# the-professor510/RSMCRT

Hardware: AMD Instinct MI355X
Metric: photon packets/sec (128^3 jmean grid, path-length deposition) (higher is better)
Workload: dtype f64

## Files before the change

include/smcrt.h:

```cpp
#ifndef SMCRT_H
#define SMCRT_H

#include <stddef.h>
#include <stdint.h>

#ifdef __cplusplus
extern "C" {
#endif

#define SMCRT_ABI_VERSION 5

typedef enum smcrt_status {
  SMCRT_OK = 0,
  SMCRT_ERR_INVALID_ARG = -1,
  SMCRT_ERR_HIP = -2,
  SMCRT_ERR_RCCL = -3,
  SMCRT_ERR_DEVICE_FAULT = -4,
  SMCRT_ERR_NO_DEVICE = -5,
  SMCRT_ERR_OOM = -6,
  SMCRT_ERR_UNSUPPORTED = -7
} smcrt_status;

typedef enum smcrt_sdf_kind {
  SMCRT_SDF_SPHERE = 1,
// ... 321 lines not shown
  int64_t lean_hazards;
} smcrt_kernel_times;

int smcrt_scene_set_timing(smcrt_scene* scene, int32_t enable);
int smcrt_scene_kernel_times(smcrt_scene* scene, smcrt_kernel_times* out);

enum {
  SMCRT_DEPOSIT_ATOMIC = 0,
  SMCRT_DEPOSIT_SORTED = 1,
  SMCRT_DEPOSIT_BUCKETS = 2
};
int smcrt_scene_deposit_regime(const smcrt_scene* scene, int32_t* regime);

int smcrt_scene_invoxel_segments(smcrt_scene* scene, int64_t* out);

int smcrt_normalise_fluence(float* grid, const smcrt_grid* g, uint64_t nphotons);

typedef enum smcrt_symmetry {
  SMCRT_SYM_NONE = 0,
  SMCRT_SYM_PRISM = 1,
  SMCRT_SYM_FLIPPED = 2,
  SMCRT_SYM_UNIFORM_SLAB = 3,
  SMCRT_SYM_NONE_ROTATIONAL = 4,
  SMCRT_SYM_ROTATIONAL_360 = 5
} smcrt_symmetry;

typedef struct smcrt_escape_config {
  int32_t symmetry;
  int32_t n[3];
  double max[3];
// ... 131 lines not shown
```

rsmcrt_amd/abi.py:

```python
import ctypes as C

SMCRT_ABI_VERSION = 5

OK = 0
ERR_INVALID_ARG = -1
ERR_HIP = -2
ERR_RCCL = -3
ERR_DEVICE_FAULT = -4
ERR_NO_DEVICE = -5
ERR_OOM = -6
ERR_UNSUPPORTED = -7

STATUS_NAMES = {
    OK: "OK", ERR_INVALID_ARG: "INVALID_ARG", ERR_HIP: "HIP_ERROR", ERR_RCCL: "RCCL_ERROR",
    ERR_DEVICE_FAULT: "DEVICE_FAULT", ERR_NO_DEVICE: "NO_DEVICE", ERR_OOM: "OUT_OF_MEMORY",
    ERR_UNSUPPORTED: "UNSUPPORTED",
}

SDF_SPHERE, SDF_BOX, SDF_TORUS, SDF_CYLINDER, SDF_TRIPRISM = 1, 2, 3, 4, 5
SDF_SEGMENT, SDF_CAPSULE, SDF_CONE, SDF_EGG, SDF_PLANE, SDF_MODEL = 6, 7, 8, 9, 10, 11
SDF_REVOLUTION, SDF_EXTRUDE, SDF_ONION, SDF_TWIST, SDF_BEND, SDF_ELONGATE, SDF_DISPLACEMENT = 12, 13, 14, 15, 16, 17, 18
DISP_SINE, DISP_EXPR = 1, 2

OP_UNION, OP_SMOOTH_UNION, OP_SUBTRACTION, OP_INTERSECTION = 0, 1, 2, 3
# ... 208 lines not shown
EXPORTED_SYMBOLS = [
    "smcrt_abi_version", "smcrt_device_count", "smcrt_last_error", "smcrt_scene_create",
    "smcrt_scene_destroy", "smcrt_scene_det_bins", "smcrt_scene_set_optprops", "smcrt_run",
    "smcrt_run_device", "smcrt_normalise_fluence", "smcrt_scene_set_timing", "smcrt_scene_kernel_times",
    "smcrt_write_data_f32", "smcrt_write_data_f64", "smcrt_write_detector", "smcrt_write_checkpoint",
    "smcrt_job_load", "smcrt_job_destroy", "smcrt_job_info", "smcrt_job_scene", "smcrt_job_metadata", "smcrt_job_run",
    "smcrt_scene_info", "smcrt_run_origins", "smcrt_scene_classify", "smcrt_escape_sym_dims", "smcrt_escape_cells",
    "smcrt_escape_map", "smcrt_escape_run", "smcrt_scene_get_optprops", "smcrt_inverse_run", "smcrt_job_load_mode",
    "smcrt_job_escape_config", "smcrt_job_inverse_config", "smcrt_job_targets", "smcrt_job_run_escape",
    "smcrt_job_run_inverse", "smcrt_scene_fence",
    "smcrt_pack_size", "smcrt_pack_host", "smcrt_unpack_host", "smcrt_comm_unique_id", "smcrt_comm_init_rank",
    "smcrt_comm_info", "smcrt_comm_destroy", "smcrt_reduce_device_tallies", "smcrt_multi_create", "smcrt_multi_info",
    "smcrt_multi_scene", "smcrt_multi_run", "smcrt_multi_accumulate", "smcrt_multi_collect",
    "smcrt_multi_device_photons", "smcrt_multi_destroy", "smcrt_job_run_devices",
    "smcrt_spectral_sample", "smcrt_scene_set_spectral", "smcrt_scene_check",
    "smcrt_scene_invoxel_segments",
    "smcrt_scene_set_path_tracking", "smcrt_scene_path_counts", "smcrt_scene_read_paths", "smcrt_write_paths",
    "smcrt_job_history_filename",
    "smcrt_scene_set_phasor", "smcrt_scene_read_phasor", "smcrt_scene_reset_phasor",
    "smcrt_displacement_compile", "smcrt_displacement_eval", "smcrt_displacement_describe",
    "smcrt_voxel_scene_create", "smcrt_scene_deposit_regime",
]
```

rsmcrt_amd/csrc/sceneplan.cpp:

```cpp
#include "sceneplan.h"

#include <algorithm>
#include <cmath>
#include <cstdlib>
#include <cstring>
#include <functional>
#include <string>

#include "dispexpr.h"
#include "hosterr.h"

namespace smcrt {
namespace {

int fail(int code, const std::string& msg) { return set_error(code, msg); }
bool is(const char* v, const char* s) { return v && std::strcmp(v, s) == 0; }

}

Knobs read_knobs() {
  Knobs k;
  auto num = [](const char* v, double d) { return v ? std::atof(v) : d; };
  if (const char* cm = std::getenv("SMCRT_COOP_MIN_TOPS")) k.coop_min_tops = std::max(1, std::atoi(cm));
  if (const char* cl = std::getenv("SMCRT_COOP_LANES")) k.coop_lanes = std::max(1, std::min(64, std::atoi(cl)));
// ... 6 lines not shown
  k.cull_grid.u_frac = num(std::getenv("SMCRT_CULL_UFRAC"), 1.0);
  k.cull_log = std::getenv("SMCRT_CULL_LOG") != nullptr;
  k.far_march = !is(std::getenv("SMCRT_FAR_MARCH"), "0");
  const char* dm = std::getenv("SMCRT_DEPOSIT");
  k.deposit_atomic = is(dm, "atomic");
  k.deposit_sorted = is(dm, "sorted");
  if (const char* pc = std::getenv("SMCRT_POOL_CAP"))
    k.pool_cap_chunks = std::max<uint64_t>(1, std::strtoull(pc, nullptr, 10) / CHUNK_RECORDS);
  const char* fp = std::getenv("SMCRT_FOLD_PRIO");
  k.fold_prio = !(fp && fp[0] == '0');
  k.fused_hist = !is(std::getenv("SMCRT_FUSED_HIST"), "0");
  const char* wsl = std::getenv("SMCRT_WS_SLOTS");
  k.ws_two_slots = wsl && wsl[0] == '2';
  const char* wi = std::getenv("SMCRT_WS_INVOXEL");
  k.ws_invoxel = wi ? (is(wi, "0") ? 0 : 1) : -1;
  const char* le = std::getenv("SMCRT_LEAN");
  k.lean_mode = le ? (is(le, "0") ? 0 : 1) : -1;
  const char* lm = std::getenv("SMCRT_DEBUG_LEAN_MARGIN");
  k.lean_debug = is(lm, "all") ? 2u : (is(lm, "0") ? 1u : 0u);
  k.verbose = std::getenv("SMCRT_VERBOSE") != nullptr;
  return k;
}

LaunchKnobs read_launch_knobs() {
  LaunchKnobs k;
#ifdef SMCRT_DIAG
  const char* dd = std::getenv("SMCRT_DIAG_DONE");
  k.diag_done = dd && dd[0] == '1';
#endif
  if (const char* wm = std::getenv("SMCRT_WATCHDOG_MS")) k.watchdog_ms = std::strtod(wm, nullptr);
// ... 241 lines not shown
  if (!p.ctab.empty() || p.cull.enabled) plan_far_march(nodes, top, n_top, grid, knobs.far_march, p);
  plan_grid_mode(grid, p);
  plan_deposit(grid, knobs, p);
  p.face_bytes = p.faces.size() * sizeof(double) + sizeof(TopProps) * (size_t)n_top;
  p.lds_faces = p.face_bytes <= MAX_FACE_BYTES;
  for (int32_t i = 1; i < n_top; ++i) p.fresnel = p.fresnel || p.h_props[i].n != p.h_props[0].n;
  {
    bool ok = p.bucketed && p.coop_lanes == 0 && grid->nx < (1 << 20) - 2 && grid->ny < (1 << 20) - 2 &&
              grid->nz < (1 << 20) - 2;
    p.ws_slots = (!knobs.ws_two_slots && lean_lds(p) + lim.ws_shared3 <= LDS_BYTES) ? 3 : 2;
    ok = ok && lean_lds(p) + (p.ws_slots == 3 ? lim.ws_shared3 : lim.ws_shared2) <= LDS_BYTES;
    p.lean_mode = knobs.lean_mode;
    p.lean_candidate = ok && !p.nested && (p.lean_mode == 1 || (p.lean_mode != 0 && n_dets == 0));
    p.lean_debug = knobs.lean_debug;
    p.ws_invoxel = knobs.ws_invoxel;
  }
  p.fold_prio = knobs.fold_prio;
  p.cull_log = knobs.cull_log;
  p.verbose = knobs.verbose;
  return SMCRT_OK;
}

int plan_voxel_scene(const uint8_t* labels, const smcrt_medium* media, int32_t n_media, const smcrt_grid* grid,
                     const smcrt_detector* dets, int32_t n_dets, const Knobs& knobs, ScenePlan* out) {
  if (!labels || !media || !grid || n_dets < 0 || (n_dets > 0 && !dets))
    return fail(SMCRT_ERR_INVALID_ARG, "voxel scene: NULL argument");
  if (n_media < 1 || n_media > 256)
    return fail(SMCRT_ERR_INVALID_ARG, "voxel scene: n_media = " + std::to_string(n_media) + " is outside 1 .. 256");
  if (grid->nx < 1 || grid->ny < 1 || grid->nz < 1 || !(grid->xmax > 0) || !(grid->ymax > 0) || !(grid->zmax > 0) ||
      !std::isfinite(grid->xmax) || !std::isfinite(grid->ymax) || !std::isfinite(grid->zmax))
// ... 63 lines not shown
```

rsmcrt_amd/csrc/sceneplan.h:

```cpp
#pragma once
#include <stdint.h>

#include <algorithm>
#include <vector>

#include "../../include/smcrt.h"
#include "transport.h"
#include "cull.h"
#include "deposit.h"

namespace smcrt {

constexpr int MAX_SLOTS = 4;
#ifndef SMCRT_DEEP_SLOT_GIB
#define SMCRT_DEEP_SLOT_GIB 24
#endif
constexpr uint64_t DEEP_SLOT_BYTES = (uint64_t)SMCRT_DEEP_SLOT_GIB << 30;

enum QueueWord : int {
  Q_STREAM0 = 0,
  Q_CALLER = MAX_SLOTS,
  Q_FAR_STEPS,
  Q_FOLD_TICKS,
  Q_LEAN_HAZARDS,
  Q_WATCHDOG,
  Q_INVOXEL,
  Q_COUNT
};
constexpr int N_QUEUES = Q_CALLER + 1;

constexpr size_t LDS_BYTES = 163840;
constexpr size_t MAX_FACE_BYTES = 40960;
constexpr uint32_t MAX_FUSED_HIST_TILES = 512;
constexpr uint64_t MAX_POOL_RECORDS = (1ull << 32) - (1ull << 28);
constexpr double POOL_SLACK = 1.15;
constexpr double DEFAULT_WATCHDOG_MS = 2000.0;

struct Knobs {
  int32_t coop_min_tops = 8;
  int32_t coop_lanes = 0;
  bool coop_tab = true;
  bool cull = true;
  CullKnobs cull_grid;
  bool cull_log = false;
  bool far_march = true;
  bool deposit_atomic = false, deposit_sorted = false;
  uint64_t pool_cap_chunks = 0;
  bool fold_prio = true;
  bool fused_hist = true;
  bool ws_two_slots = false;
  int ws_invoxel = -1;
  int lean_mode = -1;
  uint32_t lean_debug = 0;
  bool verbose = false;
};
struct LaunchKnobs {
  int32_t path_vertices = 64;
  int64_t path_max = 65536;
  double watchdog_ms = DEFAULT_WATCHDOG_MS;
  uint32_t claim_delay = 0;
  bool drop_event = false;
  bool diag_done = false;
};
struct PoolKnobs {
  int slots = 0;
  bool deep_set = false;
// ... 29 lines not shown
  double inv2[3] = {0.0, 0.0, 0.0};
  int grid_mode = 0;
  int32_t fe[3] = {0, 0, 0};
  uint32_t n_tiles = 0;
  bool force_atomic = false;
  uint64_t pool_cap_chunks = 0;
  bool bucketed = false;
  uint32_t hist_tiles = 0;
  size_t face_bytes = 0;
  bool lds_faces = false;
  bool fresnel = false;
  int ws_slots = 3;
  int lean_mode = -1;
  uint32_t lean_debug = 0;
  int ws_invoxel = -1;
  bool lean_candidate = false;
  bool fold_prio = true, cull_log = false, verbose = false;
  bool voxel = false;
  std::vector<uint8_t> labels;
};

int plan_scene(const smcrt_sdf_node* nodes, int32_t n_nodes, const int32_t* top, int32_t n_top, const smcrt_grid* grid,
               const smcrt_detector* dets, int32_t n_dets, const Knobs& knobs, const PlanLimits& lim, ScenePlan* out);

TopProps make_props(const smcrt_sdf_node& nd);

int plan_voxel_scene(const uint8_t* labels, const smcrt_medium* media, int32_t n_media, const smcrt_grid* grid,
                     const smcrt_detector* dets, int32_t n_dets, const Knobs& knobs, ScenePlan* out);
int32_t host_vox_of(double p, int32_t n, double max);
inline size_t voxel_lds(const ScenePlan& p, uint32_t dep_words) {
// ... 22 lines not shown
inline int slot_depth(const PoolKnobs& k, bool lean_or_far, uint64_t cap_bytes, uint64_t total_mem) {
  const int want = k.slots ? k.slots : (lean_or_far ? 2 : MAX_SLOTS);
  uint64_t deep = std::max<uint64_t>(DEEP_SLOT_BYTES, (uint64_t)(0.6 * (double)total_mem) / MAX_SLOTS);
  if (k.deep_set) deep = k.deep_bytes;
  return cap_bytes <= deep ? want : 2;
}
inline bool launch_binned(const ScenePlan& p, bool has_jmean, uint32_t flags) {
  return has_jmean && (flags & SMCRT_FLAG_PATHLENGTH) && !(flags & SMCRT_FLAG_SURVIVAL_BIAS) && p.n_tiles > 0 &&
         !p.force_atomic;
}
inline bool launch_lean(bool lean_ok, bool xsrc, uint32_t bucket_tiles, uint32_t flags) {
  return !xsrc && lean_ok && bucket_tiles && (flags & SMCRT_FLAG_PATHLENGTH) &&
         !(flags & (SMCRT_FLAG_SURVIVAL_BIAS | SMCRT_FLAG_TRACK_PATHS | SMCRT_FLAG_PHASOR));
}
inline bool ws_invoxel_on(int knob, bool xf) { return knob < 0 ? !xf : knob != 0; }
inline void lean_margins(uint32_t lean_debug, const smcrt_grid& g, double lo[3], double hi[3]) {
  const double eps = 1e-8, mf = (lean_debug & 3u) ? 0.0 : 2.0 * eps;
  const double mx = mf * (double)(g.nx + 2), my = mf * (double)(g.ny + 2), mz = mf * (double)(g.nz + 2);
  lo[0] = mx; lo[1] = my; lo[2] = mz;
  hi[0] = 2.0 * g.xmax - mx; hi[1] = 2.0 * g.ymax - my; hi[2] = 2.0 * g.zmax - mz;
}

}
```

rsmcrt_amd/csrc/smcrt.hip:

```cpp
#include <hip/hip_runtime.h>

#include <algorithm>
#include <cmath>
#include <cstdio>
#include <cstring>
#include <memory>
#include <mutex>
#include <string>
#include <vector>

#define SMCRT_FOLD_KERNELS
#include "../../include/smcrt.h"
#include "scene_internal.h"
#include "transport.h"
#include "deposit.h"
#include "devmem.h"
#include "hosterr.h"
#include "sceneplan.h"

using namespace smcrt;

#include "kernel_ptrs.h"


// ... 640 lines not shown

#ifdef SMCRT_DIAG
static int diag_report(hipStream_t stream, bool lean) {
  unsigned long long h[72], ht[9], hc[6];
  HIPCHK(hipStreamSynchronize(stream));
  kinst_diag_gather(h, ht, hc);
  if (lean) {
    const double wi = (double)std::max(1ull, h[20]), pt = (double)std::max(1ull, h[24]);
    std::fprintf(stderr, "[diag-ws] walker iters %llu: idle %.3f, busy lanes/iter %.1f, pending lanes/iter %.1f | "
                 "photon trips %llu: sleep %.3f, idle lanes %.1f, sync-waiting %.2f, slot-blocked %.2f, EVAL lanes "
                 "%.1f, pushes %.2f, P7 runs %.3f (lanes/run %.1f), event-waiting %.2f | producer waits %llu | event "
                 "iters %llu, lanes/iter %.1f\n",
                 h[20], h[21] / wi, h[22] / wi, h[23] / wi, h[24], h[25] / pt, h[30] / pt, h[27] / pt, h[26] / pt,
                 h[31] / pt, h[32] / pt, h[28] / pt, (double)h[29] / (double)std::max(1ull, h[28]), h[36] / pt, h[33],
                 h[34], (double)h[35] / (double)std::max(1ull, h[34]));
    const char* np[8] = {"fetch", "poll", "eval", "p3p4", "handout", "p5p6", "p7", "p8"};
    double tp = 0, tw = 0, te = 0;
    for (int i = 0; i < 8; ++i) tp += (double)h[37 + i];
    for (int i = 0; i < 4; ++i) tw += (double)h[45 + i];
    te = (double)h[49] + (double)h[50];
    std::fprintf(stderr, "[diag-ws-time] photon:");
    for (int i = 0; i < 8; ++i) std::fprintf(stderr, " %s=%.3f", np[i], (double)h[37 + i] / std::max(1.0, tp));
    std::fprintf(stderr, " | walker: claim=%.3f idle=%.3f walk=%.3f finish=%.3f | event: run=%.3f idle=%.3f | "
                 "ticks photon/walker/event %.3g/%.3g/%.3g\n", h[45] / std::max(1.0, tw), h[46] / std::max(1.0, tw),
                 h[47] / std::max(1.0, tw), h[48] / std::max(1.0, tw), h[49] / std::max(1.0, te),
                 h[50] / std::max(1.0, te), tp, tw, te);
  }
  unsigned long long lt = 0;
  for (int i = 0; i < 64; ++i) lt += h[i];
  std::fprintf(stderr, "[diag] waves %llu, longest wave %llu trips %llu ticks\n", h[70], h[68], h[69]);
// ... 65 lines not shown
  K.xmax = s->grid.xmax; K.ymax = s->grid.ymax; K.zmax = s->grid.zmax;
  K.flags = cfg->flags;
  Ch.src = *src;
  Ch.plan = plan;
  K.key0 = (uint32_t)cfg->seed;
  K.key1 = (uint32_t)(cfg->seed >> 32);
  Ch.jmean = dt.jmean; Ch.absorb = dt.absorb; Ch.emission = dt.emission;
  Ch.chunk_fill = nullptr; Ch.dep_ctl = nullptr; Ch.bin_counts = nullptr;
  Ch.bucket_tile = nullptr; Ch.bucket_fill = nullptr; Ch.tile_nb = nullptr;
  Ch.det_bins = dt.det_bins; Ch.nscatt = dt.nscatt; Ch.moments = dt.moments;
  Ch.counters = (unsigned long long*)dt.counters;
  Ch.queue = nullptr;
  Ch.far_steps = s->d_queue + Q_FAR_STEPS;
  Ch.lean_hazards = s->d_queue + Q_LEAN_HAZARDS;
  Ch.invoxel_segs = s->d_queue + Q_INVOXEL;
  Ch.lane_scratch = nullptr;
  Ch.watchdog = watchdog_word(s);
  const bool hist = (cfg->flags & SMCRT_FLAG_TRACK_PATHS) && s->path_on;
  Ch.hist_scratch = hist ? (double*)s->d_hist_scratch : nullptr;
  Ch.path_vertices = hist ? (double*)s->d_path_vertices : nullptr;
  Ch.path_headers = hist ? (smcrt_path*)s->d_path_headers : nullptr;
  Ch.path_ctl = hist ? (unsigned long long*)s->d_path_ctl : nullptr;
  Ch.hist_lanes = hist ? s->hist_lanes : 0;
  Ch.path_max = hist ? (uint64_t)s->path_cfg.max_paths : 0;
  Ch.range_first = hist ? s->path_cfg.range_first : 0;
  Ch.range_count = hist ? s->path_cfg.range_count : 0;
  Ch.hist_max_vertices = hist ? (uint32_t)s->path_cfg.max_vertices : 0;
  const bool phas = (cfg->flags & SMCRT_FLAG_PHASOR) && s->phasor_on;
  Ch.phasor = phas ? (double*)s->d_phasor : nullptr;
  Ch.phasor_fixed = phas && s->phasor_cfg.fixed_k ? 1u : 0u;
// ... 8 lines not shown
  Ch.done_base = cfg->first_photon;
  if (knobs.diag_done && diag_done_ok) {
    s->n_done = cfg->n_photons;
    HIPCHK(s->d_done.alloc(s->n_done));
    HIPCHK(hipMemsetAsync(s->d_done, 0, sizeof(unsigned long long) * s->n_done, stream));
    Ch.done_time = s->d_done;
  }
#else
  (void)stream; (void)diag_done_ok;
#endif
  Ch.watchdog_ticks = knobs.watchdog_ms > 0.0 ? (uint64_t)(knobs.watchdog_ms * (double)s->wall_khz) : 0ull;
  K.rec_pool = nullptr; K.n_chunks = 0; K.hist_tiles = 0; K.bucket_tiles = 0; K.n_buckets = 0;
  K.claim_delay = knobs.claim_delay;
  K.lean_debug = s->lean_debug | (knobs.drop_event ? 4u : 0u);
  K.ws_invoxel = ws_invoxel_on(s->ws_invoxel, s->d_lscratch != nullptr) ? 1u : 0u;
  lean_margins(K.lean_debug, s->grid, K.lean_lo, K.lean_hi);
  return SMCRT_OK;
}

static int launch(smcrt_scene* s, const smcrt_source* src, const smcrt_run_config* cfg,
                  const smcrt_device_tallies& dt, hipStream_t stream, const OriginRun* orun = nullptr) {
  if (src->kind < SMCRT_SRC_POINT || src->kind > SMCRT_SRC_APERTURE) return fail(SMCRT_ERR_INVALID_ARG, "bad source kind");
  if (cfg->n_photons == 0) return SMCRT_OK;
  const bool xsrc = src_needs_plan(src) || orun || s->nested;
  SrcPlan plan;
  std::memset(&plan, 0, sizeof plan);
  if (xsrc) {
    std::vector<double> px, py, pc;
    const char* perr = "";
    const int pst = build_src_plan(src, &s->grid, &plan, px, py, pc, &perr);
// ... 380 lines not shown
                                                            : SMCRT_DEPOSIT_SORTED;
  return SMCRT_OK;
}

int smcrt_scene_invoxel_segments(smcrt_scene* s, int64_t* out) {
  if (!s || !out) return fail(SMCRT_ERR_INVALID_ARG, "NULL argument");
  if (const int vst = smcrt::scene_refuse_voxel(s, "smcrt_scene_invoxel_segments")) return vst;
  std::lock_guard<std::mutex> g(s->mu);
  HIPCHK(hipSetDevice(s->device));
  unsigned long long n = 0;
  HIPCHK(hipMemcpy(&n, s->d_queue + Q_INVOXEL, sizeof(n), hipMemcpyDeviceToHost));
  *out = (int64_t)n;
  return SMCRT_OK;
}

static void release_paths(smcrt_scene* s) {
  s->path_on = false;
  s->d_hist_scratch.reset(); s->d_path_vertices.reset(); s->d_path_headers.reset(); s->d_path_ctl.reset();
  s->hist_lanes = 0;
}

int smcrt_scene_set_path_tracking(smcrt_scene* s, const smcrt_path_config* cfg) {
  g_last_error.clear();
  if (!s) return fail(SMCRT_ERR_INVALID_ARG, "scene is NULL");
  if (const int vst = smcrt::scene_refuse_voxel(s, "path tracking")) return vst;
  if (cfg) {
    if (cfg->max_vertices < 2 || cfg->max_vertices > 1024)
      return fail(SMCRT_ERR_INVALID_ARG, "path tracking: max_vertices must lie in 2 .. 1024");
    if (cfg->max_paths < 1) return fail(SMCRT_ERR_INVALID_ARG, "path tracking: max_paths must be >= 1");
    if (cfg->range_count > UINT64_MAX - cfg->range_first)
// ... 165 lines not shown
```

rsmcrt_amd/csrc/transport.h:

```cpp
#pragma once
#include <hip/hip_runtime.h>
#include <stdint.h>

#include <type_traits>

#include "../../include/smcrt.h"
#include "detmath.h"
#include "geometry.h"
#include "srcplan.h"
#include "cull.h"

namespace smcrt {

constexpr int64_t MAX_EMIT_TRIES = 100000;
constexpr int64_t MAX_HOP_ITERS = 1000000;
constexpr int64_t MAX_MARCH_ITERS = 10000000;
constexpr int64_t MAX_GLANCE_ITERS = 100000;
constexpr int64_t MAX_DDA_ITERS = 10000000;
constexpr int MAX_RENORM_ITERS = 64;
constexpr int64_t MAX_INTERACTIONS = 100000000;

#define SMCRT_DDA_PER_ITER 3
#define SMCRT_FETCH_CHUNK 64
#define SMCRT_EVENT_LANES 16
// ... 33 lines not shown
  SrcPlan plan;
  double* hist_scratch;
  double* path_vertices;
  smcrt_path* path_headers;
  unsigned long long* path_ctl;
  uint64_t hist_lanes;
  uint64_t path_max;
  uint64_t range_first, range_count;
  uint32_t hist_max_vertices;
  uint32_t phasor_fixed;
  double* phasor;
  double phasor_k;
  const uint8_t* vox_labels;
  uint32_t vox_n_media;
  uint32_t vox_reserved;
};

enum : uint32_t {
  WDOG_PHOTON_WAVE = 1,
  WDOG_RING = 2,
  WDOG_EVENT_QUEUE = 3,
  WDOG_BUCKET = 4
};
__device__ __forceinline__ bool watchdog_expired(const KCold* __restrict__ C, uint64_t t0, uint32_t site) {
  const uint64_t budget = C->watchdog_ticks;
  if (budget == 0 || __builtin_amdgcn_s_memrealtime() - t0 <= budget) return false;
  atomicCAS(C->watchdog, 0u, site | ((blockIdx.x + 1u) << 8));
  return true;
}

// ... 9 lines not shown
  int32_t n_prog, n_top, n_dets;
  int32_t coop_lanes;
  int32_t nx, ny, nz;
  uint32_t flags;
  double xmax, ymax, zmax;
  double inv2x, inv2y, inv2z;
  int32_t fex, fey, fez;
  uint32_t key0, key1;
  unsigned long long* rec_pool;
  uint32_t n_chunks;
  uint32_t hist_tiles;
  uint32_t bucket_tiles, n_buckets;
  uint32_t claim_delay;
  uint32_t lean_debug;
  uint32_t ws_invoxel;
  double lean_lo[3], lean_hi[3];
  const CullGrid* __restrict__ cull;
  const double* __restrict__ ctab;
  double fm_err, fm_step;
};

template <int GM>
__device__ __forceinline__ double cell_floor(double p, int32_t n, double max, double inv, int32_t fe) {
  if constexpr (GM == 2) return floor(ldexp(p, -fe));
  const double a = (double)n * p;
  return floor(GM >= 1 ? a * inv : (inv != 0.0 ? a * inv : a / (2.0 * max)));
}
__device__ __forceinline__ int32_t cvt_sat_i32(double f) {
  int32_t r;
  asm("v_cvt_i32_f64 %0, %1" : "=v"(r) : "v"(f));
// ... 1283 lines not shown
```

rsmcrt_amd/csrc/ws.h:

```cpp
#pragma once
#include <hip/hip_runtime.h>
#include <stdint.h>

#include "invoxel.h"
#include "lean.h"

namespace smcrt {

#ifndef SMCRT_WS_PHOTON_WAVES
#define SMCRT_WS_PHOTON_WAVES 8
#endif
#ifndef SMCRT_WS_EVENT_WAVES
#define SMCRT_WS_EVENT_WAVES 1
#endif
#ifndef SMCRT_WS_DDA
#define SMCRT_WS_DDA 2
#endif
#ifndef SMCRT_WS_WAVES
#define SMCRT_WS_WAVES 16
#endif
#ifndef SMCRT_WS_KBOUNDS_PLAIN
#define SMCRT_WS_KBOUNDS_PLAIN 0
#endif
#ifndef SMCRT_WS_START_CELLS
#define SMCRT_WS_START_CELLS 1
#endif
#ifndef SMCRT_WS_INVOXEL_LDS
#define SMCRT_WS_INVOXEL_LDS 0
#endif
constexpr uint32_t WS_NO_VOX = 0xFFFFFFFFu;
constexpr int WS_WAVES = SMCRT_WS_WAVES;
constexpr int WS_THREADS = 64 * WS_WAVES;
constexpr int WS_PW = SMCRT_WS_PHOTON_WAVES;
constexpr int WS_EW = SMCRT_WS_EVENT_WAVES;
static_assert(WS_PW >= 1 && WS_EW >= 1 && WS_PW + WS_EW < WS_WAVES, "a block needs all three roles");
constexpr uint32_t WS_NPL = 64u * WS_PW;
constexpr uint32_t ws_pow2(uint32_t v) { return v <= 1 ? 1 : 2 * ws_pow2((v + 1) / 2); }
constexpr uint32_t WS_EQ = ws_pow2(WS_NPL);
constexpr uint32_t WS_CONSUMED = 1u << 12;
constexpr uint32_t WS_SEQ_MASK = 0xFFFFF000u;
__device__ __forceinline__ uint32_t ws_tick(uint32_t t) { return ((t + 1u) & 0x7FFFFu) << 13; }

enum : int { SG_OX = 0, SG_OY, SG_OZ, SG_DX, SG_DY, SG_DZ, SG_LEN, SG_N };
// ... 32 lines not shown
__host__ __device__ constexpr size_t ws_scratch_bytes(size_t lanes) {
  return lanes * (WX_ND * sizeof(double) + WXI_N * sizeof(uint32_t));
}

template <class S>
__device__ __forceinline__ void ws_count(S* sh, int c) {
  const uint64_t m = __ballot(1);
  if ((int)(threadIdx.x & 63) == __builtin_ctzll(m)) atomicAdd(&sh->wctr[threadIdx.x >> 6][c], (uint32_t)__popcll(m));
}

template <class S>
__device__ __forceinline__ uint32_t ws_busy(S* sh, uint32_t pl) {
  return __hip_atomic_load(&sh->busy[pl], __ATOMIC_ACQUIRE, __HIP_MEMORY_SCOPE_WORKGROUP);
}

__device__ __forceinline__ uint32_t ws_load(uint32_t* p) {
  return __hip_atomic_load(p, __ATOMIC_RELAXED, __HIP_MEMORY_SCOPE_WORKGROUP);
}


#ifdef SMCRT_ASM_MARKERS
#define WS_MARK(i) asm volatile("; @@LPHASE " #i)
#else
#define WS_MARK(i) do {} while (0)
#endif
#ifdef SMCRT_DIAG
enum : int { WD_WITERS = 20, WD_WIDLE, WD_WBUSY, WD_WPEND, WD_PTRIPS, WD_PSLEEP, WD_PBLOCKED, WD_PWAIT, WD_P7,
             WD_P7LANES, WD_PIDLE, WD_ELANES, WD_PUSH, WD_PRODWAIT, WD_EITERS, WD_ELANESRUN, WD_PEVQ,
             WD_TP_FETCH, WD_TP_POLL, WD_TP_EVAL, WD_TP_P34, WD_TP_HAND, WD_TP_P56, WD_TP_P7, WD_TP_P8,
             WD_TW_CLAIM, WD_TW_IDLE, WD_TW_WALK, WD_TW_FIN, WD_TE_RUN, WD_TE_IDLE, WD_N };
static_assert(WD_N <= 64, "g_diag[64..] belongs to transport_kernel");
#define WSDIAG(i, v) (wd[(i) - WD_WITERS] += (uint64_t)(v))
#define WST(i)                                                \
  do {                                                        \
    const uint64_t now_ = __builtin_amdgcn_s_memtime();       \
    wd[(i) - WD_WITERS] += now_ - tprev;                      \
    tprev = now_;                                             \
  } while (0)
#else
#define WSDIAG(i, v) do {} while (0)
#define WST(i) do {} while (0)
#endif

template <bool LDS_FACES, int GM, bool XF, uint32_t SL, bool IV>
__global__ __launch_bounds__(WS_THREADS) __attribute__((amdgpu_waves_per_eu(4))) void ws_kernel(
// ... 36 lines not shown
    sh->iv_acc[i] = 0.0;
    sh->iv_vox[i] = WS_NO_VOX;
#endif
  }
  for (uint32_t i = threadIdx.x; i < WS_RING; i += WS_THREADS) sh->meta[i] = 0;
  for (uint32_t i = threadIdx.x; i < WS_EQ; i += WS_THREADS) sh->evq[i] = 0;
  if (threadIdx.x == 0) {
    sh->head = sh->tail = 0;
    sh->ev_head = sh->ev_tail = 0;
    sh->alive = WS_PW;
    sh->abort_ = 0;
  }
  __syncthreads();

  uint32_t w_iters = 0, w_sdf = 0, w_dep = 0, hazards = 0;
  uint32_t r_upd = 0, r_scat = 0, r_tau = 0, r_abs = 0, r_inv = 0;
#ifdef SMCRT_DIAG
  uint64_t wd[WD_N - WD_WITERS] = {};
  uint64_t tprev = __builtin_amdgcn_s_memtime();
#endif
  if (wv < WS_PW) {
    WS_MARK(1);
    const bool test_kernel = (K.flags & SMCRT_FLAG_TEST_KERNEL) != 0;
    const bool records_on = (K.flags & SMCRT_FLAG_RECORD_PHOTONS) != 0 && C->records != nullptr;
    const uint32_t pl = threadIdx.x;
#define WLU(f) (sh->lu[(f)][pl])
    const double mf = (K.lean_debug & 3u) ? 0.0 : 2.0 * eps;
    const double mx0 = mf * (double)(K.nx + 2), my0 = mf * (double)(K.ny + 2), mz0 = mf * (double)(K.nz + 2);
    const double ex0 = 2.0 * K.xmax - mx0, ey0 = 2.0 * K.ymax - my0, ez0 = 2.0 * K.zmax - mz0;
    const bool defer_all = (K.lean_debug & 3u) == 2u;
    bool drop_event = (K.lean_debug & 4u) && blockIdx.x == 0 && pl == 0;
    const bool invoxel_on = IV && K.ws_invoxel != 0 && (K.flags & SMCRT_FLAG_PATHLENGTH) != 0;
#if SMCRT_WS_INVOXEL_LDS
#define WS_IV_ACC (sh->iv_acc[pl])
#define WS_IV_VOX (sh->iv_vox[pl])
#else
    double iv_acc = 0.0;
    uint32_t iv_vox = WS_NO_VOX;
#define WS_IV_ACC iv_acc
#define WS_IV_VOX iv_vox
#endif
    auto iv_flush = [&]() {
      const uint32_t av = WS_IV_VOX;
      if (av != WS_NO_VOX) {
        atomic_add_nr(C->jmean + av, WS_IV_ACC);
        WS_IV_ACC = 0.0;
// ... 50 lines not shown
          const uint64_t rank = __popcll(need & ((1ull << lane_id) - 1ull));
          if (P.st == ST_FETCH && rank < take) {
            P.rng.init(C->first_photon + chunk_base + rank);
            sh->ev_pid[0][pl] = P.rng.pid_lo; sh->ev_pid[1][pl] = P.rng.pid_hi;
            P.st = ST_EMIT;
          }
          chunk_base += take;
          chunk_left -= take;
          need = __ballot(P.st == ST_FETCH);
        }
        if (!more && P.st == ST_FETCH) P.st = ST_IDLE;
        const uint64_t live = __ballot(P.st != ST_IDLE);
        if (live == 0) break;
      }
      WST(WD_TP_FETCH);
      if (P.has(LF_EVQ)) {
        const uint32_t code = __hip_atomic_load(&sh->ev_code[pl], __ATOMIC_ACQUIRE, __HIP_MEMORY_SCOPE_WORKGROUP);
        if (code & EV_DONE) {
          P.clr(LF_EVQ);
          P.rng.draws = sh->ev_draws[pl];
          P.rng.cached = sh->ev_cached[pl];
          if (P.st == ST_EMIT) {
            P.pos = v3(sh->seg[P.seq][SG_OX][pl], sh->seg[P.seq][SG_OY][pl], sh->seg[P.seq][SG_OZ][pl]);
            P.dir = v3(sh->ev_dir[0][pl], sh->ev_dir[1][pl], sh->ev_dir[2][pl]);
            P.clr(LF_TFLAG);
            P.layer = (int32_t)(code & 0xFFFFu);
            P.xcell = vox_of<GM>(P.pos.x, K.nx, K.xmax, K.inv2x, K.fex);
            P.ycell = vox_of<GM>(P.pos.y, K.ny, K.ymax, K.inv2y, K.fey);
            P.zcell = vox_of<GM>(P.pos.z, K.nz, K.zmax, K.inv2z, K.fez);
            P.set(LF_CELLS);
// ... 28 lines not shown
          } else if (code & EV_ABSORB) {
            P.set(LF_TFLAG);
            P.st = ST_ABSORB;
          } else {
            if (code & EV_RUNAWAY) P.set(LF_FAULT | LF_TFLAG);
            P.dir = v3(sh->ev_dir[0][pl], sh->ev_dir[1][pl], sh->ev_dir[2][pl]);
            P.tau = sh->ev_tau[pl];
            P.taurun = 0.0;
            P.hop = 0;
            P.st = ST_H0;
            t2_entry();
            p8();
          }
        }
      }
      WSDIAG(WD_PTRIPS, 1);
      WSDIAG(WD_PIDLE, __popcll(__ballot(P.st == ST_IDLE)));
      WSDIAG(WD_PWAIT, __popcll(__ballot(P.has(LF_WAIT))));
      WSDIAG(WD_PEVQ, __popcll(__ballot(P.has(LF_EVQ))));

      WST(WD_TP_POLL);
      const bool have = (P.f & (LF_PEND | LF_REQ | LF_WAIT)) == LF_PEND;
      EvalOut R;
      R.minabs = R.minv = R.va = R.vb = 0.0; R.maxloc = 0;
      if (__ballot(have)) {
        const bool mask_le = test_kernel && P.st == ST_LAYER;
        const V3 q = (P.st == ST_H1 || P.st == ST_G0) ? P.pos + smul(P.d, P.dir) : P.pos;
        R = eval_sdfs(nodes, prog, K.n_prog, q, mask_le, 0, 0);
        const bool counted = P.st == ST_H0 || P.st == ST_H1 || P.st == ST_H3 || P.st == ST_M1 || P.st == ST_G0;
        w_sdf += __popcll(__ballot(have && counted)) * (uint32_t)K.n_top;
        WSDIAG(WD_ELANES, __popcll(__ballot(have)));
        if (have) P.clr(LF_PEND);
      }

      WST(WD_TP_EVAL);
      if (have && (P.st == ST_H0 || P.st == ST_H3 || P.st == ST_M1)) {
        const uint32_t st0 = P.st;
        P.minabs = R.minabs;
        const bool small = st0 == ST_H0 && R.minabs < eps;
        const bool out = st0 != ST_H0 && R.minv > 0.0;
        if (out) P.set(LF_TFLAG);
        if (st0 == ST_H0) P.loopc = 0;
        const bool done = P.taurun >= P.tau || P.has(LF_TFLAG);
        P.d = small ? R.minabs + 2.0 * eps : R.minabs;
        uint32_t ns = st0 == ST_M1 ? (out ? (uint32_t)ST_B0 : (uint32_t)ST_M0) : (done ? (uint32_t)ST_T2END : (uint32_t)ST_M0);
        if (small) { ns = ST_H1; P.set(LF_PEND); }
// ... 102 lines not shown
          if constexpr (!IV) {
            old = v3(P.pos.x + K.xmax, P.pos.y + K.ymax, P.pos.z + K.zmax);
            ci = cell_of<GM>(old.x, K.nx, K.xmax, K.inv2x, K.fex);
            cj = cell_of<GM>(old.y, K.ny, K.ymax, K.inv2y, K.fey);
            ck = cell_of<GM>(old.z, K.nz, K.zmax, K.inv2z, K.fez);
          }
          if (P.has(LF_MOVE_FWD)) P.pos = P.pos + smul(P.d, P.dir);
          else if (P.has(LF_MOVE_BACK)) P.pos = P.pos - smul(P.d, P.dir);
          P.clr(LF_REQ | LF_MOVE_FWD | LF_MOVE_BACK);
          if (ci == -1 || cj == -1 || ck == -1) {
            P.set(LF_TFLAG | LF_CELLS);
            P.xcell = ci; P.ycell = cj; P.zcell = ck;
          } else {
            const double len = P.d;
            const V3 e = v3(old.x + P.dir.x * len, old.y + P.dir.y * len, old.z + P.dir.z * len);
            constexpr bool KB = XF || SMCRT_WS_KBOUNDS_PLAIN;
            const double mx = KB ? K.lean_lo[0] : mx0, my = KB ? K.lean_lo[1] : my0, mz = KB ? K.lean_lo[2] : mz0;
            const double ex = KB ? K.lean_hi[0] : ex0, ey = KB ? K.lean_hi[1] : ey0, ez = KB ? K.lean_hi[2] : ez0;
            const bool inside = old.x >= mx && old.x <= ex && old.y >= my && old.y <= ey && old.z >= mz &&
                                old.z <= ez && e.x >= mx && e.x <= ex && e.y >= my && e.y <= ey && e.z >= mz &&
                                e.z <= ez;
            push = true;
            sync = !inside && !defer_all;
#if SMCRT_WS_START_CELLS
            sh->pcell[pl][slot] = lean_pack(ci, cj, ck);
#endif
            if constexpr (GM != 2) {
              const bool in_cell = face<GM>(xf, ci - 1, K.fex) <= old.x && old.x <= face<GM>(xf, ci, K.fex) &&
                                   face<GM>(yf, cj - 1, K.fey) <= old.y && old.y <= face<GM>(yf, cj, K.fey) &&
                                   face<GM>(zf, ck - 1, K.fez) <= old.z && old.z <= face<GM>(zf, ck, K.fez);
              if (!in_cell) sync = true;
            }
          }
// ... 21 lines not shown
              WSDIAG(WD_PRODWAIT, 1);
              __builtin_amdgcn_s_sleep(1);
              if (!t0) t0 = __builtin_amdgcn_s_memrealtime();
              else if (watchdog_expired(C, t0, WDOG_RING)) break;
            }
            __hip_atomic_store(&sh->meta[ix], pl | (slot << 9) | (sync ? (1u << 11) : 0u) | ws_tick(t),
                               __ATOMIC_RELEASE, __HIP_MEMORY_SCOPE_WORKGROUP);
            P.seq = P.seq + 1 == WS_SLOTS ? 0u : P.seq + 1;
            P.clr(LF_CELLS);
            if (sync) P.set(LF_WAIT);
          }
        }
      }

      WST(WD_TP_HAND);
      if (P.has(LF_WAIT) && !(ws_busy(sh, pl) & (1u << ((P.seq + WS_SLOTS - 1) % WS_SLOTS)))) {
        const unsigned long long w = sh->pcell[pl][(P.seq + WS_SLOTS - 1) % WS_SLOTS];
        P.xcell = lean_cell(w, 0); P.ycell = lean_cell(w, 1); P.zcell = lean_cell(w, 2);
        P.set(LF_CELLS);
        if (w & LEAN_TFLAG) P.set(LF_TFLAG);
        if (w & LEAN_FAULT) P.set(LF_FAULT);
        P.clr(LF_WAIT);
      }
      const bool free_ = !(P.f & (LF_REQ | LF_WAIT));
      if (free_ && (P.st == ST_H2 || P.st == ST_B0 || P.st == ST_X1)) {
        if (P.st == ST_X1) {
          P.taurun = P.taurun + P.d * props[P.layer - 1].kappa;
          if (XF && P.has(LF_SSP)) P.pos = v3(X[WX_SSP * xs], X[(WX_SSP + 1) * xs], X[(WX_SSP + 2) * xs]);
          else P.pos = P.pos + smul(P.d, P.dir);
          P.clr(LF_SSP);
// ... 473 lines not shown
    close_buckets(K, C, WB, w_dep - overflow, overflow);
  }
  WS_MARK(16);
  {
    unsigned long long* const counters = C->counters;
    const uint32_t hz = wave_sum_u32(hazards);
    const uint32_t n_upd = wave_sum_u32(r_upd), n_scat = wave_sum_u32(r_scat), n_tau = wave_sum_u32(r_tau),
                   n_abs = wave_sum_u32(r_abs), n_inv = wave_sum_u32(r_inv);
    if (lane_id == 0) {
      if (hz) {
        atomicAdd(C->dep_ctl + 5, hz);
        atomicAdd(C->lean_hazards, (unsigned long long)hz);
      }
      if (C->dep_ctl && n_upd) atomicAdd(C->dep_ctl + 6, n_upd);
      if (n_inv) atomicAdd(C->invoxel_segs, (unsigned long long)n_inv);
      if (counters) {
        const uint32_t* c = sh->wctr[wv];
        const uint32_t v[SMCRT_NCOUNTERS] = {c[LC_PHOTONS], c[LC_RETRIES], n_scat,        n_abs,          w_sdf,
                                             w_dep + n_inv, n_upd,         n_tau,          c[LC_FRES],     c[LC_REFL],
                                             c[LC_BABORT],  c[LC_FAULTS] + hz, c[LC_DRAWS], c[LC_HITS],   c[LC_ESCAPED],
                                             w_iters};
        for (int i = 0; i < SMCRT_NCOUNTERS; ++i)
          if (v[i]) atomicAdd(counters + i, (unsigned long long)v[i]);
      }
      double* const nscatt = C->nscatt;
      if (nscatt && n_scat) atomic_add_nr(nscatt, (double)n_scat);
    }
  }
#ifdef SMCRT_DIAG
  if (lane_id == 0)
// ... 9 lines not shown
```

rsmcrt_amd/engine.py:

```python
from __future__ import annotations

import ctypes as C
import os
import threading

import numpy as np

from . import abi
from .scene import Mono, VoxelScene, detector_array
from .tallies import Result

LIB_PATH = os.environ.get("SMCRT_LIB") or os.path.join(os.path.dirname(os.path.abspath(__file__)), "libsmcrt.so")
_lock = threading.Lock()
_lib = None


class SmcrtError(RuntimeError):
    pass


def load_library(path: str = LIB_PATH):
    global _lib
    with _lock:
        if _lib is not None:
# ... 294 lines not shown
        g = self.grid
        out = np.zeros((g.nz, g.ny, g.nx), dtype=np.complex128)
        _check(load_library().smcrt_scene_read_phasor(self._h, out.ctypes.data_as(C.POINTER(C.c_double))))
        return out

    def reset_phasor(self):
        _check(load_library().smcrt_scene_reset_phasor(self._h))

    def invoxel_segments(self) -> int:
        fn = load_library().smcrt_scene_invoxel_segments
        fn.argtypes = [C.c_void_p, C.POINTER(C.c_int64)]
        n = C.c_int64()
        _check(fn(self._h, C.byref(n)))
        return n.value


def pack_layout(grid, n_det_bins: int, fields: int) -> abi.PackLayout:
    lay = abi.PackLayout()
    lay.n_voxels, lay.n_det_bins, lay.fields = grid.nx * grid.ny * grid.nz, int(n_det_bins), int(fields)
    return lay


def pack_result(res: Result, fields: int) -> np.ndarray:
    L = load_library()
    lay = pack_layout(res.grid, sum(res.det_sizes), fields)
    n = C.c_int64()
    _check(L.smcrt_pack_size(C.byref(lay), C.byref(n)))
    buf = np.zeros(n.value)
    t = res.tallies()
    _check(L.smcrt_pack_host(C.byref(lay), C.byref(t), buf.ctypes.data_as(C.POINTER(C.c_double))))
# ... 118 lines not shown
```

Baseline: 272.4 million.

## Run multiple evaluation rounds per producer trip in work-stealing loop

New measurement: 274.5 million, median of 6. No clear change (+0.8%).

```diff
diff --git a/include/smcrt.h b/include/smcrt.h
--- a/include/smcrt.h
+++ b/include/smcrt.h
@@ -359,6 +359,8 @@
 
 int smcrt_scene_invoxel_segments(smcrt_scene* scene, int64_t* out);
 
+int smcrt_scene_ws_rounds(smcrt_scene* scene, int64_t out[2]);
+
 int smcrt_normalise_fluence(float* grid, const smcrt_grid* g, uint64_t nphotons);
 
 typedef enum smcrt_symmetry {
diff --git a/rsmcrt_amd/abi.py b/rsmcrt_amd/abi.py
--- a/rsmcrt_amd/abi.py
+++ b/rsmcrt_amd/abi.py
@@ -246,7 +246,7 @@
     "smcrt_multi_scene", "smcrt_multi_run", "smcrt_multi_accumulate", "smcrt_multi_collect",
     "smcrt_multi_device_photons", "smcrt_multi_destroy", "smcrt_job_run_devices",
     "smcrt_spectral_sample", "smcrt_scene_set_spectral", "smcrt_scene_check",
-    "smcrt_scene_invoxel_segments",
+    "smcrt_scene_invoxel_segments", "smcrt_scene_ws_rounds",
     "smcrt_scene_set_path_tracking", "smcrt_scene_path_counts", "smcrt_scene_read_paths", "smcrt_write_paths",
     "smcrt_job_history_filename",
     "smcrt_scene_set_phasor", "smcrt_scene_read_phasor", "smcrt_scene_reset_phasor",
diff --git a/rsmcrt_amd/csrc/sceneplan.cpp b/rsmcrt_amd/csrc/sceneplan.cpp
--- a/rsmcrt_amd/csrc/sceneplan.cpp
+++ b/rsmcrt_amd/csrc/sceneplan.cpp
@@ -44,6 +44,7 @@
   k.ws_two_slots = wsl && wsl[0] == '2';
   const char* wi = std::getenv("SMCRT_WS_INVOXEL");
   k.ws_invoxel = wi ? (is(wi, "0") ? 0 : 1) : -1;
+  if (const char* wr = std::getenv("SMCRT_WS_ROUNDS")) k.ws_rounds = std::max(1, std::min(4, std::atoi(wr)));
   const char* le = std::getenv("SMCRT_LEAN");
   k.lean_mode = le ? (is(le, "0") ? 0 : 1) : -1;
   const char* lm = std::getenv("SMCRT_DEBUG_LEAN_MARGIN");
@@ -315,6 +316,7 @@
     p.lean_candidate = ok && !p.nested && (p.lean_mode == 1 || (p.lean_mode != 0 && n_dets == 0));
     p.lean_debug = knobs.lean_debug;
     p.ws_invoxel = knobs.ws_invoxel;
+    p.ws_rounds = knobs.ws_rounds;
   }
   p.fold_prio = knobs.fold_prio;
   p.cull_log = knobs.cull_log;
diff --git a/rsmcrt_amd/csrc/sceneplan.h b/rsmcrt_amd/csrc/sceneplan.h
--- a/rsmcrt_amd/csrc/sceneplan.h
+++ b/rsmcrt_amd/csrc/sceneplan.h
@@ -25,6 +25,8 @@
   Q_LEAN_HAZARDS,
   Q_WATCHDOG,
   Q_INVOXEL,
+  Q_WS_TRIPS,
+  Q_WS_ROUNDS,
   Q_COUNT
 };
 constexpr int N_QUEUES = Q_CALLER + 1;
@@ -50,6 +52,7 @@
   bool fused_hist = true;
   bool ws_two_slots = false;
   int ws_invoxel = -1;
+  int ws_rounds = 0;
   int lean_mode = -1;
   uint32_t lean_debug = 0;
   bool verbose = false;
@@ -109,6 +112,7 @@
   int lean_mode = -1;
   uint32_t lean_debug = 0;
   int ws_invoxel = -1;
+  int ws_rounds = 0;
   bool lean_candidate = false;
   bool fold_prio = true, cull_log = false, verbose = false;
   bool voxel = false;
@@ -161,6 +165,8 @@
          !(flags & (SMCRT_FLAG_SURVIVAL_BIAS | SMCRT_FLAG_TRACK_PATHS | SMCRT_FLAG_PHASOR));
 }
 inline bool ws_invoxel_on(int knob, bool xf) { return knob < 0 ? !xf : knob != 0; }
+constexpr int WS_ROUNDS_PLAIN = 1, WS_ROUNDS_XF = 3;
+inline uint32_t ws_rounds_for(int knob, bool xf) { return (uint32_t)(knob > 0 ? knob : (xf ? WS_ROUNDS_XF : WS_ROUNDS_PLAIN)); }
 inline void lean_margins(uint32_t lean_debug, const smcrt_grid& g, double lo[3], double hi[3]) {
   const double eps = 1e-8, mf = (lean_debug & 3u) ? 0.0 : 2.0 * eps;
   const double mx = mf * (double)(g.nx + 2), my = mf * (double)(g.ny + 2), mz = mf * (double)(g.nz + 2);
diff --git a/rsmcrt_amd/csrc/smcrt.hip b/rsmcrt_amd/csrc/smcrt.hip
--- a/rsmcrt_amd/csrc/smcrt.hip
+++ b/rsmcrt_amd/csrc/smcrt.hip
@@ -678,6 +678,8 @@
                  h[20], h[21] / wi, h[22] / wi, h[23] / wi, h[24], h[25] / pt, h[30] / pt, h[27] / pt, h[26] / pt,
                  h[31] / pt, h[32] / pt, h[28] / pt, (double)h[29] / (double)std::max(1ull, h[28]), h[36] / pt, h[33],
                  h[34], (double)h[35] / (double)std::max(1ull, h[34]));
+    std::fprintf(stderr, "[diag-ws-rounds] rounds/trip %.3f, EVAL lanes/trip by round: %.2f %.2f %.2f %.2f\n", h[51] / pt,
+                 h[52] / pt, h[53] / pt, h[54] / pt, h[55] / pt);
     const char* np[8] = {"fetch", "poll", "eval", "p3p4", "handout", "p5p6", "p7", "p8"};
     double tp = 0, tw = 0, te = 0;
     for (int i = 0; i < 8; ++i) tp += (double)h[37 + i];
@@ -773,6 +775,7 @@
   Ch.far_steps = s->d_queue + Q_FAR_STEPS;
   Ch.lean_hazards = s->d_queue + Q_LEAN_HAZARDS;
   Ch.invoxel_segs = s->d_queue + Q_INVOXEL;
+  Ch.ws_rounds = s->d_queue + Q_WS_TRIPS;
   Ch.lane_scratch = nullptr;
   Ch.watchdog = watchdog_word(s);
   const bool hist = (cfg->flags & SMCRT_FLAG_TRACK_PATHS) && s->path_on;
@@ -811,6 +814,7 @@
   K.claim_delay = knobs.claim_delay;
   K.lean_debug = s->lean_debug | (knobs.drop_event ? 4u : 0u);
   K.ws_invoxel = ws_invoxel_on(s->ws_invoxel, s->d_lscratch != nullptr) ? 1u : 0u;
+  K.ws_rounds = ws_rounds_for(s->ws_rounds, s->d_lscratch != nullptr);
   lean_margins(K.lean_debug, s->grid, K.lean_lo, K.lean_hi);
   return SMCRT_OK;
 }
@@ -1221,6 +1225,19 @@
   return SMCRT_OK;
 }
 
+int smcrt_scene_ws_rounds(smcrt_scene* s, int64_t out[2]) {
+  if (!s || !out) return fail(SMCRT_ERR_INVALID_ARG, "NULL argument");
+  if (const int vst = smcrt::scene_refuse_voxel(s, "smcrt_scene_ws_rounds")) return vst;
+  std::lock_guard<std::mutex> g(s->mu);
+  HIPCHK(hipSetDevice(s->device));
+  static_assert(Q_WS_ROUNDS == Q_WS_TRIPS + 1, "read together");
+  unsigned long long n[2] = {0, 0};
+  HIPCHK(hipMemcpy(n, s->d_queue + Q_WS_TRIPS, sizeof(n), hipMemcpyDeviceToHost));
+  out[0] = (int64_t)n[0];
+  out[1] = (int64_t)n[1];
+  return SMCRT_OK;
+}
+
 static void release_paths(smcrt_scene* s) {
   s->path_on = false;
   s->d_hist_scratch.reset(); s->d_path_vertices.reset(); s->d_path_headers.reset(); s->d_path_ctl.reset();
diff --git a/rsmcrt_amd/csrc/transport.h b/rsmcrt_amd/csrc/transport.h
--- a/rsmcrt_amd/csrc/transport.h
+++ b/rsmcrt_amd/csrc/transport.h
@@ -71,6 +71,7 @@
   const uint8_t* vox_labels;
   uint32_t vox_n_media;
   uint32_t vox_reserved;
+  unsigned long long* ws_rounds;
 };
 
 enum : uint32_t {
@@ -110,6 +111,7 @@
   uint32_t claim_delay;
   uint32_t lean_debug;
   uint32_t ws_invoxel;
+  uint32_t ws_rounds;
   double lean_lo[3], lean_hi[3];
   const CullGrid* __restrict__ cull;
   const double* __restrict__ ctab;
diff --git a/rsmcrt_amd/csrc/ws.h b/rsmcrt_amd/csrc/ws.h
--- a/rsmcrt_amd/csrc/ws.h
+++ b/rsmcrt_amd/csrc/ws.h
@@ -19,14 +19,14 @@
 #ifndef SMCRT_WS_WAVES
 #define SMCRT_WS_WAVES 16
 #endif
-#ifndef SMCRT_WS_KBOUNDS_PLAIN
-#define SMCRT_WS_KBOUNDS_PLAIN 0
-#endif
 #ifndef SMCRT_WS_START_CELLS
 #define SMCRT_WS_START_CELLS 1
 #endif
 #ifndef SMCRT_WS_INVOXEL_LDS
 #define SMCRT_WS_INVOXEL_LDS 0
+#endif
+#ifndef SMCRT_WS_ROUND_MIN
+#define SMCRT_WS_ROUND_MIN 1
 #endif
 constexpr uint32_t WS_NO_VOX = 0xFFFFFFFFu;
 constexpr int WS_WAVES = SMCRT_WS_WAVES;
@@ -89,6 +89,11 @@
   return __hip_atomic_load(&sh->busy[pl], __ATOMIC_ACQUIRE, __HIP_MEMORY_SCOPE_WORKGROUP);
 }
 
+__device__ __forceinline__ uint32_t ws_fresh(uint32_t v) {
+  asm volatile("" : "+v"(v));
+  return v;
+}
+
 __device__ __forceinline__ uint32_t ws_load(uint32_t* p) {
   return __hip_atomic_load(p, __ATOMIC_RELAXED, __HIP_MEMORY_SCOPE_WORKGROUP);
 }
@@ -103,7 +108,8 @@
 enum : int { WD_WITERS = 20, WD_WIDLE, WD_WBUSY, WD_WPEND, WD_PTRIPS, WD_PSLEEP, WD_PBLOCKED, WD_PWAIT, WD_P7,
              WD_P7LANES, WD_PIDLE, WD_ELANES, WD_PUSH, WD_PRODWAIT, WD_EITERS, WD_ELANESRUN, WD_PEVQ,
              WD_TP_FETCH, WD_TP_POLL, WD_TP_EVAL, WD_TP_P34, WD_TP_HAND, WD_TP_P56, WD_TP_P7, WD_TP_P8,
-             WD_TW_CLAIM, WD_TW_IDLE, WD_TW_WALK, WD_TW_FIN, WD_TE_RUN, WD_TE_IDLE, WD_N };
+             WD_TW_CLAIM, WD_TW_IDLE, WD_TW_WALK, WD_TW_FIN, WD_TE_RUN, WD_TE_IDLE,
+             WD_PROUNDS, WD_RHAVE0, WD_N = WD_RHAVE0 + 4 };
 static_assert(WD_N <= 64, "g_diag[64..] belongs to transport_kernel");
 #define WSDIAG(i, v) (wd[(i) - WD_WITERS] += (uint64_t)(v))
 #define WST(i)                                                \
@@ -170,6 +176,7 @@
   __syncthreads();
 
   uint32_t w_iters = 0, w_sdf = 0, w_dep = 0, hazards = 0;
+  uint32_t w_trips = 0, w_rounds = 0;
   uint32_t r_upd = 0, r_scat = 0, r_tau = 0, r_abs = 0, r_inv = 0;
 #ifdef SMCRT_DIAG
   uint64_t wd[WD_N - WD_WITERS] = {};
@@ -181,11 +188,9 @@
     const bool records_on = (K.flags & SMCRT_FLAG_RECORD_PHOTONS) != 0 && C->records != nullptr;
     const uint32_t pl = threadIdx.x;
 #define WLU(f) (sh->lu[(f)][pl])
-    const double mf = (K.lean_debug & 3u) ? 0.0 : 2.0 * eps;
-    const double mx0 = mf * (double)(K.nx + 2), my0 = mf * (double)(K.ny + 2), mz0 = mf * (double)(K.nz + 2);
-    const double ex0 = 2.0 * K.xmax - mx0, ey0 = 2.0 * K.ymax - my0, ez0 = 2.0 * K.zmax - mz0;
     const bool defer_all = (K.lean_debug & 3u) == 2u;
     bool drop_event = (K.lean_debug & 4u) && blockIdx.x == 0 && pl == 0;
+    const uint32_t n_rounds = K.ws_rounds;
     const bool invoxel_on = IV && K.ws_invoxel != 0 && (K.flags & SMCRT_FLAG_PATHLENGTH) != 0;
 #if SMCRT_WS_INVOXEL_LDS
 #define WS_IV_ACC (sh->iv_acc[pl])
@@ -266,6 +271,11 @@
         if (live == 0) break;
       }
       WST(WD_TP_FETCH);
+      ++w_trips;
+      uint32_t round = 0;
+#pragma nounroll
+      for (;;) {
+      ++w_rounds;
       if (P.has(LF_EVQ)) {
         const uint32_t code = __hip_atomic_load(&sh->ev_code[pl], __ATOMIC_ACQUIRE, __HIP_MEMORY_SCOPE_WORKGROUP);
         if (code & EV_DONE) {
@@ -324,10 +334,13 @@
           }
         }
       }
-      WSDIAG(WD_PTRIPS, 1);
-      WSDIAG(WD_PIDLE, __popcll(__ballot(P.st == ST_IDLE)));
-      WSDIAG(WD_PWAIT, __popcll(__ballot(P.has(LF_WAIT))));
-      WSDIAG(WD_PEVQ, __popcll(__ballot(P.has(LF_EVQ))));
+      if (round == 0) {
+        WSDIAG(WD_PTRIPS, 1);
+        WSDIAG(WD_PIDLE, __popcll(__ballot(P.st == ST_IDLE)));
+        WSDIAG(WD_PWAIT, __popcll(__ballot(P.has(LF_WAIT))));
+        WSDIAG(WD_PEVQ, __popcll(__ballot(P.has(LF_EVQ))));
+      }
+      WSDIAG(WD_PROUNDS, 1);
 
       WST(WD_TP_POLL);
       const bool have = (P.f & (LF_PEND | LF_REQ | LF_WAIT)) == LF_PEND;
@@ -340,6 +353,7 @@
         const bool counted = P.st == ST_H0 || P.st == ST_H1 || P.st == ST_H3 || P.st == ST_M1 || P.st == ST_G0;
         w_sdf += __popcll(__ballot(have && counted)) * (uint32_t)K.n_top;
         WSDIAG(WD_ELANES, __popcll(__ballot(have)));
+        WSDIAG(WD_RHAVE0 + round, __popcll(__ballot(have)));
         if (have) P.clr(LF_PEND);
       }
 
@@ -472,9 +486,8 @@
           } else {
             const double len = P.d;
             const V3 e = v3(old.x + P.dir.x * len, old.y + P.dir.y * len, old.z + P.dir.z * len);
-            constexpr bool KB = XF || SMCRT_WS_KBOUNDS_PLAIN;
-            const double mx = KB ? K.lean_lo[0] : mx0, my = KB ? K.lean_lo[1] : my0, mz = KB ? K.lean_lo[2] : mz0;
-            const double ex = KB ? K.lean_hi[0] : ex0, ey = KB ? K.lean_hi[1] : ey0, ez = KB ? K.lean_hi[2] : ez0;
+            const double mx = K.lean_lo[0], my = K.lean_lo[1], mz = K.lean_lo[2];
+            const double ex = K.lean_hi[0], ey = K.lean_hi[1], ez = K.lean_hi[2];
             const bool inside = old.x >= mx && old.x <= ex && old.y >= my && old.y <= ey && old.z >= mz &&
                                 old.z <= ez && e.x >= mx && e.x <= ex && e.y >= my && e.y <= ey && e.z >= mz &&
                                 e.z <= ez;
@@ -526,6 +539,11 @@
       }
 
       WST(WD_TP_HAND);
+      if (round + 1 >= n_rounds) break;
+      if (__popcll(__ballot((P.f & (LF_PEND | LF_REQ | LF_WAIT)) == LF_PEND)) < SMCRT_WS_ROUND_MIN) break;
+      ++round;
+      }
+      const uint32_t pl = ws_fresh(threadIdx.x);
       if (P.has(LF_WAIT) && !(ws_busy(sh, pl) & (1u << ((P.seq + WS_SLOTS - 1) % WS_SLOTS)))) {
         const unsigned long long w = sh->pcell[pl][(P.seq + WS_SLOTS - 1) % WS_SLOTS];
         P.xcell = lean_cell(w, 0); P.ycell = lean_cell(w, 1); P.zcell = lean_cell(w, 2);
@@ -1029,6 +1047,10 @@
       }
       if (C->dep_ctl && n_upd) atomicAdd(C->dep_ctl + 6, n_upd);
       if (n_inv) atomicAdd(C->invoxel_segs, (unsigned long long)n_inv);
+      if (w_trips) {
+        atomicAdd(C->ws_rounds, (unsigned long long)w_trips);
+        atomicAdd(C->ws_rounds + 1, (unsigned long long)w_rounds);
+      }
       if (counters) {
         const uint32_t* c = sh->wctr[wv];
         const uint32_t v[SMCRT_NCOUNTERS] = {c[LC_PHOTONS], c[LC_RETRIES], n_scat,        n_abs,          w_sdf,
diff --git a/rsmcrt_amd/engine.py b/rsmcrt_amd/engine.py
--- a/rsmcrt_amd/engine.py
+++ b/rsmcrt_amd/engine.py
@@ -332,6 +332,13 @@
         _check(fn(self._h, C.byref(n)))
         return n.value
 
+    def ws_rounds(self):
+        fn = load_library().smcrt_scene_ws_rounds
+        fn.argtypes = [C.c_void_p, C.POINTER(C.c_int64)]
+        out = (C.c_int64 * 2)()
+        _check(fn(self._h, out))
+        return out[0], out[1]
+
 
 def pack_layout(grid, n_det_bins: int, fields: int) -> abi.PackLayout:
     lay = abi.PackLayout()
```
